# ikt-luh/Demo-Learned-Point-Cloud-Compression

Measured on AMD Instinct MI355X. Metric: point-cloud frames/sec encode+decode @1M pts, higher is better.
Workload: dtype f32

## Files before the change

demo-learned-point-cloud-compression_amd/csrc/codec.hip:

```cpp
#include "common.h"

#include <string.h>

#include <algorithm>
#include <atomic>
#include <chrono>
#include <deque>
#include <exception>
#include <new>
#include <map>
#include <memory>
#include <string>
#include <condition_variable>
#include <functional>
#include <mutex>
#include <thread>
#include <vector>

namespace {

double now_s() {
  return std::chrono::duration<double>(std::chrono::steady_clock::now().time_since_epoch()).count();
}

constexpr int64_t kHashBuildMax = 60000;
constexpr int64_t kMaxLatentRows = (int64_t)1 << 27;
constexpr int64_t kEarlyZSymbols = (int64_t)1 << 22;

int log2i(int ts) {
  int s = 0;
  while ((1 << s) < ts) ++s;
  return s;
}

struct Tensor {
  int dtype = 0;
  std::vector<int64_t> dims;
  const uint8_t* data = nullptr;
  size_t nbytes = 0;
  int64_t numel() const {
    int64_t n = 1;
    for (int64_t d : dims) n *= d;
    return n;
  }
  const float* f32() const { return reinterpret_cast<const float*>(data); }
  const int32_t* i32() const { return reinterpret_cast<const int32_t*>(data); }
};

struct DevPool {
  struct Block {
    char* p;
    size_t cap, off;
  };
  std::vector<Block> blocks;
  void reset() {
    if (blocks.size() > 32) {
      size_t total = 0;
      for (auto& b : blocks) total += b.cap;
      release();
      char* p = nullptr;
      if (hipMalloc((void**)&p, total) == hipSuccess) blocks.push_back({p, total, 0});
    }
    for (auto& b : blocks) b.off = 0;
  }
  void* alloc(size_t bytes) {
    bytes = (std::max<size_t>(bytes, 1) + 255) & ~(size_t)255;
    for (auto& b : blocks)
      if (b.cap - b.off >= bytes) {
        void* r = b.p + b.off;
        b.off += bytes;
        return r;
      }
    const size_t cap = std::max<size_t>(bytes, (size_t)64 << 20);
    char* p = nullptr;
    if (hipMalloc((void**)&p, cap) != hipSuccess) {
      pcc_set_error("codec pool: hipMalloc(%zu) failed", cap);
      return nullptr;
    }
    blocks.push_back({p, cap, bytes});
    return p;
  }
  void release() {
    for (auto& b : blocks) (void)hipFree(b.p);
// ... 41 lines not shown
  uint32_t* keep = nullptr;
  int32_t* keep_remap = nullptr;
};

struct Feat {
  CS* cs = nullptr;
  float* f = nullptr;
  int c = 0;
  const uint32_t* rows = nullptr;
};

}

struct PccWorkers {
  std::vector<std::thread> th;
  std::vector<std::function<void()>> job;
  std::vector<char> busy;
  std::mutex m;
  std::condition_variable cv_job, cv_done;
  bool stop = false;

  void ensure(int n) {
    std::unique_lock<std::mutex> lk(m);
    while ((int)th.size() < n) {
      const int i = (int)th.size();
      job.resize((size_t)i + 1);
      busy.resize((size_t)i + 1, 0);
      th.emplace_back([this, i]() {
        std::unique_lock<std::mutex> l(m);
        for (;;) {
          cv_job.wait(l, [&] { return stop || busy[i]; });
          if (stop) return;
          std::function<void()> f = std::move(job[i]);
          l.unlock();
          try {
            f();
          } catch (...) {
          }
          l.lock();
          busy[i] = 0;
          cv_done.notify_all();
        }
      });
    }
  }
  void run(int i, std::function<void()> f) {
    {
      std::lock_guard<std::mutex> lk(m);
      job[i] = std::move(f);
      busy[i] = 1;
    }
    cv_job.notify_all();
  }
  void wait_range(int lo, int hi) {
    std::unique_lock<std::mutex> lk(m);
    cv_done.wait(lk, [&] {
      for (int i = lo; i < hi && i < (int)busy.size(); ++i)
        if (busy[i]) return false;
      return true;
    });
  }
  void wait_all() {
    std::unique_lock<std::mutex> lk(m);
    cv_done.wait(lk, [&] {
      for (char b : busy)
        if (b) return false;
      return true;
    });
  }
  ~PccWorkers() {
    {
      std::lock_guard<std::mutex> lk(m);
      stop = true;
    }
    cv_job.notify_all();
    for (auto& t : th)
      if (t.joinable()) t.join();
  }
};

struct WorkersGuard {
  PccWorkers* w;
  ~WorkersGuard() { if (w) w->wait_all(); }
};

struct pcc_codec {
  pcc_ctx* ctx = nullptr;
  int device = 0;
  std::vector<uint8_t> blob;
  std::map<std::string, Tensor> t;
  std::map<std::string, float*> dev;
  int c_y = 32, c_z = 32;
  PccRansTables* gc_tables = nullptr;
  PccRansTables* eb_tables = nullptr;
  int container_version = 0;
  int seek_points = 0;
  struct ScaleSlot {
    std::vector<double> key;
    float* dev = nullptr;
    size_t cap = 0;
  } scale_slot[2];
  pcc_rans_dev *gc_dev = nullptr, *eb_dev = nullptr;
  PccWorkers workers;
  DevPool pool;
  Pinned pin_keys, pin_occ, pin_zsym, pin_ysym, pin_yidx, pin_flag, pin_dec, pin_up;
  hipStream_t up_stream = nullptr;
  hipStream_t side_stream = nullptr;
  pcc_ctx* side_ctx = nullptr;
  hipEvent_t up_done = nullptr;
  std::vector<hipEvent_t> events;
  size_t events_used = 0;
  std::deque<CS> sets;
  std::vector<std::vector<uint8_t>> out;
  int32_t* rec_coords = nullptr;
  float* rec_colors = nullptr;
  int64_t rec_n = 0;
  std::vector<int64_t> rec_offsets;
  bool rec_i16 = false;
  int16_t* rec_xyz16 = nullptr;
  float* rec_rgbp = nullptr;
  Pinned pin_out;
  hipEvent_t out_pts = nullptr;
  std::atomic<int> widen_status{0};
};

void octree_root(uint64_t first, uint64_t last, int key_shift, int* depth, int32_t origin[3]) {
  const uint64_t mask48 = ((uint64_t)1 << 48) - 1;
  const uint64_t a = (first & mask48) >> key_shift, b = (last & mask48) >> key_shift;
  const uint64_t diff = a ^ b;
  int d = 1;
  if (diff) d = (63 - __builtin_clzll(diff)) / 3 + 1;
  const uint64_t corner = (a >> (3 * d)) << (3 * d);
  const int bias = 32768 >> (key_shift / 3);
  auto compact = [](uint64_t v) {
    int r = 0;
    for (int i = 0; i < 16; ++i) r |= (int)((v >> (3 * i)) & 1) << i;
    return r;
  };
  *depth = d;
  origin[0] = compact(corner >> 2) - bias;
  origin[1] = compact(corner >> 1) - bias;
  origin[2] = compact(corner) - bias;
}


namespace {

#define CODEC_ALLOC(var, type, count)                                        \
  type* var = (type*)cd->pool.alloc(sizeof(type) * (size_t)(count));         \
  if (!var) return PCC_E_NOMEM

const Tensor* find(pcc_codec* cd, const std::string& name) {
  auto it = cd->t.find(name);
  if (it == cd->t.end()) {
    pcc_set_error("codec: checkpoint has no tensor '%s'", name.c_str());
    return nullptr;
  }
  return &it->second;
}

CS* new_set(pcc_codec* cd, uint64_t* keys, int64_t n, int stride, int n_batch) {
  cd->sets.emplace_back();
  CS* s = &cd->sets.back();
  s->keys = keys;
  s->n = n;
  s->stride = stride;
  s->n_batch = n_batch;
  return s;
}

int keys_of(pcc_codec* cd, CS* s, uint64_t** out);

int offsets_of(pcc_codec* cd, CS* s, const std::vector<int64_t>** out) {
  if (s->offsets.empty()) {
    if (s->n_batch == 1) {
      s->offsets = {0, s->n};
    } else if (s->gen_parent) {
      const std::vector<int64_t>* po;
      PCC_TRY(offsets_of(cd, s->gen_parent, &po));
      s->offsets.resize(po->size());
      for (size_t i = 0; i < po->size(); ++i) s->offsets[i] = 8 * (*po)[i];
    } else {
      s->offsets.assign((size_t)s->n_batch + 1, 0);
      PCC_TRY(pcc_batch_offsets(cd->ctx, s->keys, s->n, s->n_batch, s->offsets.data()));
    }
  }
  *out = &s->offsets;
  return PCC_OK;
}

int down_of(pcc_codec* cd, CS* s) {
  if (s->down) return PCC_OK;
// ... 333 lines not shown
}

struct Reader {
  const uint8_t* p;
  int64_t len, pos = 0;
  bool bad = false;
  int32_t be32() {
    if (pos + 4 > len) { bad = true; return 0; }
    const uint32_t u = ((uint32_t)p[pos] << 24) | ((uint32_t)p[pos + 1] << 16) | ((uint32_t)p[pos + 2] << 8) | p[pos + 3];
    pos += 4;
    return (int32_t)u;
  }
  double be_f64() {
    if (pos + 8 > len) { bad = true; return 0; }
    uint64_t u = 0;
    for (int i = 0; i < 8; ++i) u = (u << 8) | p[pos + i];
    pos += 8;
    double d;
    memcpy(&d, &u, 8);
    return d;
  }
  const uint8_t* bytes(int64_t n) {
    if (n < 0 || pos + n > len) { bad = true; return nullptr; }
    const uint8_t* r = p + pos;
    pos += n;
    return r;
  }
};

int rans_encode_grow(const int32_t* sym, const int32_t* idx, int64_t n, const Tensor* cdf, const Tensor* len,
                     const Tensor* off, std::vector<uint8_t>* out) {
  int64_t cap = 2 * n + 4096, got = 0;
  int rc = PCC_OK;
  for (int attempt = 0; attempt < 2; ++attempt) {
    out->resize((size_t)cap);
    rc = pcc_rans_encode(sym, idx, n, cdf->i32(), (int)cdf->dims[1], len->i32(), off->i32(), (int)cdf->dims[0],
                         out->data(), cap, &got);
    if (rc != PCC_E_NOMEM) break;
    cap = 48 * n + 4096;
  }
  if (rc == PCC_OK) out->resize((size_t)got);
  return rc;
}

}


static void warm_copy_paths(pcc_codec* cd) {
  hipStream_t st = cd->ctx->stream;
  const size_t big = (size_t)1 << 20;
  uint8_t *d = nullptr, *h = nullptr;
  if (hipMalloc((void**)&d, 2 * big) != hipSuccess) return;
  if (hipHostMalloc((void**)&h, 2 * big, hipHostMallocDefault) == hipSuccess) {
    for (int rep = 0; rep < 2; ++rep) {
      for (size_t bytes : {(size_t)64, (size_t)4096, (size_t)65536, big}) {
        for (int k = 0; k < 4; ++k) {
          (void)hipMemcpyAsync(h + (size_t)k * (big / 4), d + (size_t)k * (big / 4), std::min(bytes, big / 4), hipMemcpyDeviceToHost, st);
          (void)hipMemcpyAsync(d + big + (size_t)k * (big / 4), h + big + (size_t)k * (big / 4), std::min(bytes, big / 4),
                               hipMemcpyHostToDevice, st);
        }
        (void)hipMemcpy2DAsync(h, big / 4, d, big / 4, std::min(bytes, big / 4), 3, hipMemcpyDeviceToHost, st);
        (void)hipMemcpy2DAsync(h + big, big / 4, d + big, big / 4, std::min(bytes, big / 4) / 2 + 1, 3, hipMemcpyDeviceToHost, st);
      }
      (void)hipMemsetAsync(d, 0, 4096, st);
      (void)hipMemcpyAsync(d + big, d, 65536, hipMemcpyDeviceToDevice, st);
    }
    (void)hipStreamSynchronize(st);
    (void)hipHostFree(h);
  }
  (void)hipFree(d);
  (void)hipGetLastError();
}

extern "C" pcc_codec* pcc_codec_create(const void* h_ckpt, size_t n, int device, void* stream) {
  if (!h_ckpt || n < 8 || memcmp(h_ckpt, "PCCW", 4) != 0) {
    pcc_set_error("pcc_codec_create: not a PCCW checkpoint blob");
    return nullptr;
  }
  pcc_ctx* ctx = pcc_create(device, stream);
  if (!ctx) return nullptr;
  pcc_codec* cd = new pcc_codec();
  cd->ctx = ctx;
  cd->device = device;
  cd->blob.assign((const uint8_t*)h_ckpt, (const uint8_t*)h_ckpt + n);
  const uint8_t* p = cd->blob.data();
  size_t pos = 4;
  auto fail = [&](const char* why) -> pcc_codec* {
    pcc_set_error("pcc_codec_create: malformed checkpoint (%s)", why);
    pcc_destroy(cd->ctx);
    delete cd;
    return nullptr;
  };
  uint32_t count;
  memcpy(&count, p + pos, 4);
  pos += 4;
  for (uint32_t i = 0; i < count; ++i) {
    if (pos + 2 > n) return fail("truncated");
    uint16_t nl;
    memcpy(&nl, p + pos, 2);
    pos += 2;
    if (pos + nl + 2 > n) return fail("truncated name");
    std::string name((const char*)p + pos, nl);
    pos += nl;
    Tensor t;
    t.dtype = p[pos];
    const int nd = p[pos + 1];
    pos += 2;
    if (pos + 4 * (size_t)nd + 8 > n) return fail("truncated dims");
    for (int d = 0; d < nd; ++d) {
      uint32_t v;
      memcpy(&v, p + pos, 4);
      pos += 4;
      t.dims.push_back(v);
    }
    uint64_t nb;
    memcpy(&nb, p + pos, 8);
    pos += 8;
    pos = (pos + 7) & ~(size_t)7;
    if (pos + nb > n || nb != (uint64_t)t.numel() * 4) return fail("bad tensor size");
    t.data = p + pos;
    t.nbytes = nb;
    pos = (pos + nb + 7) & ~(size_t)7;
    cd->t[name] = t;
  }
  for (auto& kv : cd->t) {
    const std::string& k = kv.first;
    const bool is_wb = (k.size() > 7 && k.compare(k.size() - 7, 7, ".weight") == 0) ||
                       (k.size() > 5 && k.compare(k.size() - 5, 5, ".bias") == 0);
    const bool is_tab = k == "entropy_bottleneck.medians" || k == "gaussian_conditional.scale_table";
    if ((!is_wb && !is_tab) || k.compare(0, 8, "scale_nn") == 0 || kv.second.dtype != 0) continue;
    float* d = nullptr;
    if (hipMalloc((void**)&d, std::max<size_t>(kv.second.nbytes, 4)) != hipSuccess ||
        hipMemcpy(d, kv.second.data, kv.second.nbytes, hipMemcpyHostToDevice) != hipSuccess) {
      pcc_set_error("pcc_codec_create: upload of '%s' failed", k.c_str());
      pcc_destroy(cd->ctx);
      delete cd;
      return nullptr;
    }
    cd->dev[k] = d;
  }
  for (auto& kv : cd->t) {
    const std::string& k = kv.first;
    const Tensor& t = kv.second;
    if (k.size() <= 7 || k.compare(k.size() - 7, 7, ".weight") != 0 || t.dtype != 0 || t.dims.size() != 3) continue;
    const std::string layer = k.substr(0, k.size() - 7);
    const bool is_up = layer.find(".up") != std::string::npos;
    if (is_up && t.dims[0] == 8 && t.dims[1] == 32 && t.dims[2] == 32 && cd->dev.count(k))
      (void)pcc_conv_prepare(ctx, cd->dev[k], 8, 32, 32);
    if (!is_up && (t.dims[0] == 27 || t.dims[0] == 8) && t.dims[1] % 16 == 0 && t.dims[2] % 16 == 0 && t.dims[1] <= 128 &&
        t.dims[2] <= 256 && cd->dev.count(k)) {
      if (pcc_conv_prepare(ctx, cd->dev[k], (int)t.dims[0], (int)t.dims[1], (int)t.dims[2]) != PCC_OK) {
        for (auto& d : cd->dev) (void)hipFree(d.second);
        pcc_destroy(cd->ctx);
        delete cd;
        return nullptr;
      }
    }
    if (is_up && layer.compare(0, 4, "g_s.") == 0 && t.dims[0] == 8 && t.dims[1] == 32 && t.dims[2] == 32 &&
        cd->t.count(layer + ".bias")) {
      std::vector<float> wp((size_t)t.numel()), bp(32);
      const float* bsrc = cd->t[layer + ".bias"].f32();
      for (int64_t r = 0; r < 8 * 32; ++r)
        for (int j = 0; j < 32; ++j) wp[(size_t)r * 32 + j] = t.f32()[r * 32 + pcc_conv16_perm(j)];
      for (int j = 0; j < 32; ++j) bp[j] = bsrc[pcc_conv16_perm(j)];
      float *dw = nullptr, *db = nullptr;
      if (hipMalloc((void**)&dw, wp.size() * 4) != hipSuccess || hipMalloc((void**)&db, 128) != hipSuccess ||
// ... 14 lines not shown
  }
  static const char* need[] = {"g_a.conv0.weight", "g_a.conv3.weight", "h_a.conv0.weight", "h_s.conv0.weight",
                               "g_s.color.weight", "entropy_bottleneck.quantized_cdf",
                               "gaussian_conditional.quantized_cdf", "gaussian_conditional.scale_table",
                               "entropy_bottleneck.medians", "entropy_model.offsets_ab", "entropy_model.eps"};
  for (const char* k : need)
    if (!cd->t.count(k)) {
      pcc_set_error("pcc_codec_create: checkpoint has no tensor '%s'", k);
      for (auto& kv : cd->dev) (void)hipFree(kv.second);
      pcc_destroy(cd->ctx);
      delete cd;
      return nullptr;
    }
  cd->c_y = (int)cd->t["g_a.conv3.weight"].dims[2];
  cd->c_z = (int)cd->t["entropy_bottleneck.medians"].dims[0];
  {
    const Tensor *gc_cdf = find(cd, "gaussian_conditional.quantized_cdf"), *gc_len = find(cd, "gaussian_conditional.cdf_length"),
                 *gc_off = find(cd, "gaussian_conditional.offset");
    if (gc_cdf && gc_len && gc_off)
      cd->gc_tables = pcc_rans_tables_build(gc_cdf->i32(), (int)gc_cdf->dims[1], gc_len->i32(), gc_off->i32(),
                                            (int)gc_cdf->dims[0]);
    if (!cd->gc_tables) {
      for (auto& kv : cd->dev) (void)hipFree(kv.second);
      pcc_destroy(cd->ctx);
      delete cd;
      return nullptr;
    }
    const Tensor *eb_cdf = find(cd, "entropy_bottleneck.quantized_cdf"), *eb_len = find(cd, "entropy_bottleneck.cdf_length"),
                 *eb_off = find(cd, "entropy_bottleneck.offset");
    cd->gc_dev = pcc_rans_dev_create(gc_cdf->i32(), (int)gc_cdf->dims[1], gc_len->i32(), gc_off->i32(), (int)gc_cdf->dims[0]);
    if (eb_cdf && eb_len && eb_off)
      cd->eb_tables = pcc_rans_tables_build(eb_cdf->i32(), (int)eb_cdf->dims[1], eb_len->i32(), eb_off->i32(),
                                            (int)eb_cdf->dims[0]);
    if (eb_cdf && eb_len && eb_off)
      cd->eb_dev = pcc_rans_dev_create(eb_cdf->i32(), (int)eb_cdf->dims[1], eb_len->i32(), eb_off->i32(), (int)eb_cdf->dims[0]);
  }
  warm_copy_paths(cd);
  return cd;
}

extern "C" int pcc_codec_set_seek_points(pcc_codec* cd, int pieces) {
  PCC_REQUIRE(cd, PCC_E_ARG, "pcc_codec_set_seek_points: null codec");
  PCC_REQUIRE(pieces == 0 || (pieces >= 2 && pieces <= 64), PCC_E_ARG, "pcc_codec_set_seek_points: %d pieces (0, or 2 .. 64)", pieces);
  cd->seek_points = pieces;
  return PCC_OK;
}

static void seek_indexes(int64_t n, int pieces, std::vector<int64_t>* out) {
  out->clear();
  if (pieces < 2 || n < 65536) return;
  for (int k = 1; k < pieces; ++k) {
    const int64_t i = (n * k / pieces) & ~(int64_t)63;
    if (i > 0 && i < n && (out->empty() || i > out->back())) out->push_back(i);
  }
}

extern "C" int pcc_codec_set_container_version(pcc_codec* cd, int version) {
  PCC_REQUIRE(cd, PCC_E_ARG, "pcc_codec_set_container_version: null codec");
  PCC_REQUIRE(version == 0 || version == 1, PCC_E_ARG, "pcc_codec_set_container_version: version %d (0 or 1)", version);
  PCC_REQUIRE(version == 0 || (cd->gc_dev && cd->eb_dev), PCC_E_ARG,
              "pcc_codec_set_container_version: the checkpoint's CDF tables have no device form");
  cd->container_version = version;
  return PCC_OK;
}

extern "C" void pcc_codec_destroy(pcc_codec* cd) {
  if (!cd) return;
  if (cd->ctx) (void)pcc_sync(cd->ctx);
  for (auto& kv : cd->dev) (void)hipFree(kv.second);
  for (auto& sl : cd->scale_slot)
    if (sl.dev) (void)hipFree(sl.dev);
  pcc_rans_tables_free(cd->gc_tables);
  pcc_rans_tables_free(cd->eb_tables);
  pcc_rans_dev_destroy(cd->gc_dev);
  pcc_rans_dev_destroy(cd->eb_dev);
  cd->pool.release();
  if (cd->up_stream) {
    (void)hipStreamSynchronize(cd->up_stream);
    (void)hipStreamDestroy(cd->up_stream);
  }
  if (cd->side_ctx) pcc_destroy(cd->side_ctx);
  if (cd->side_stream) (void)hipStreamDestroy(cd->side_stream);
  if (cd->up_done) (void)hipEventDestroy(cd->up_done);
  if (cd->out_pts) (void)hipEventDestroy(cd->out_pts);
  for (hipEvent_t e : cd->events) (void)hipEventDestroy(e);
  for (Pinned* p : {&cd->pin_keys, &cd->pin_occ, &cd->pin_zsym, &cd->pin_ysym, &cd->pin_yidx, &cd->pin_flag, &cd->pin_dec,
                    &cd->pin_up, &cd->pin_out})
    p->release();
  pcc_destroy(cd->ctx);
  delete cd;
}

extern "C" pcc_ctx* pcc_codec_ctx(pcc_codec* cd) { return cd ? cd->ctx : nullptr; }

#define PCC_MAX_FRAMES_ARG 32
struct FrameTab {
  const void* pts[PCC_MAX_FRAMES_ARG];
  const void* cols[PCC_MAX_FRAMES_ARG];
  long long off[PCC_MAX_FRAMES_ARG + 1];
  int nf, pts_i16, cols_f64;
};
struct HostFrames {
  const void* const* pts;
  const void* const* cols;
};

__device__ __forceinline__ int frame_of(const FrameTab& t, long long i) {
  int f = 0;
  while (f + 1 < t.nf && i >= t.off[f + 1]) ++f;
  return f;
}

__global__ __launch_bounds__(256) void k_frames_keys(FrameTab t, int64_t n, uint64_t* __restrict__ keys,
                                                     int32_t* __restrict__ flag) {
  const int64_t i = (int64_t)blockIdx.x * blockDim.x + threadIdx.x;
  if (i >= n) return;
  const int f = frame_of(t, i);
  const int64_t j = i - t.off[f];
  int x, y, z;
  if (t.pts_i16) {
    const int16_t* p = (const int16_t*)t.pts[f] + 3 * j;
    x = p[0]; y = p[1]; z = p[2];
  } else {
    const int32_t* p = (const int32_t*)t.pts[f] + 3 * j;
    x = p[0]; y = p[1]; z = p[2];
    const bool bad = (x < -32768) | (x > 32767) | (y < -32768) | (y > 32767) | (z < -32768) | (z > 32767);
    if (bad) atomicOr(flag, 1);
  }
  keys[i] = pcc_morton(f, x, y, z);
}

__global__ void k_frame_end_keys(FrameTab t, const uint64_t* __restrict__ keys, uint64_t* __restrict__ out) {
  const int f = threadIdx.x;
  if (f >= t.nf) return;
  const bool any = t.off[f + 1] > t.off[f];
  out[2 * f] = any ? keys[t.off[f]] : 0ull;
  out[2 * f + 1] = any ? keys[t.off[f + 1] - 1] : 0ull;
}

__global__ __launch_bounds__(256) void k_frames_feats(FrameTab t, const uint32_t* __restrict__ perm, int64_t n,
                                                      float4* __restrict__ feats) {
  const int64_t i = (int64_t)blockIdx.x * blockDim.x + threadIdx.x;
  if (i >= n) return;
  const long long src = perm[i];
  const int f = frame_of(t, src);
  const int64_t j = src - t.off[f];
  float r, g, b;
  if (t.cols_f64) {
    const double* c = (const double*)t.cols[f] + 3 * j;
    r = (float)c[0]; g = (float)c[1]; b = (float)c[2];
  } else {
    const float* c = (const float*)t.cols[f] + 3 * j;
    r = c[0]; g = c[1]; b = c[2];
  }
  feats[i] = make_float4(1.0f, r, g, b);
}

struct UploadPiece {
  size_t off;
  const void* src;
  size_t count;
  int f64;
};
constexpr int kUploadThreads = 4;
constexpr size_t kUploadPieceBytes = (size_t)1 << 20;

static void upload_pieces(std::vector<UploadPiece>* out, size_t base, const void* src, size_t n_bytes_out, int f64) {
  for (size_t o = 0; o < n_bytes_out; o += kUploadPieceBytes) {
    const size_t len = std::min(kUploadPieceBytes, n_bytes_out - o);
    if (f64)
      out->push_back({base + o, (const double*)src + o / 4, len / 4, 1});
    else
      out->push_back({base + o, (const char*)src + o, len, 0});
  }
}

static void upload_run(pcc_codec* cd, const std::vector<UploadPiece>& pieces, char* stage, char* dev, hipStream_t stream,
                       std::atomic<int>* status) {
  cd->workers.ensure(kUploadThreads);
  const int device = cd->device;
  for (int w = 0; w < kUploadThreads; ++w)
    cd->workers.run(w, [&pieces, stage, dev, stream, status, device, w]() {
      if (stream && hipSetDevice(device) != hipSuccess) status->store(1);
      for (size_t i = (size_t)w; i < pieces.size(); i += kUploadThreads) {
        const UploadPiece& p = pieces[i];
        size_t bytes = p.count;
        if (p.f64) {
          float* d = (float*)(stage + p.off);
          const double* sp = (const double*)p.src;
          for (size_t j = 0; j < p.count; ++j) d[j] = (float)sp[j];
          bytes = p.count * 4;
        } else {
          memcpy(stage + p.off, p.src, p.count);
        }
        if (stream && hipMemcpyAsync(dev + p.off, stage + p.off, bytes, hipMemcpyHostToDevice, stream) != hipSuccess)
          status->store(1);
      }
    });
}

static int begin_call(pcc_codec* cd) {
  PCC_HIP(hipSetDevice(cd->device));
  PCC_TRY(pcc_sync(cd->ctx));
  if (cd->up_stream) PCC_HIP(hipStreamSynchronize(cd->up_stream));
  if (cd->side_stream) PCC_HIP(hipStreamSynchronize(cd->side_stream));
  cd->pool.reset();
  cd->events_used = 0;
  cd->sets.clear();
  return PCC_OK;
}

template <class F>
static int timed(double* clock, F&& stage) {
  const double t0 = now_s();
  const int rc = stage();
  *clock += now_s() - t0;
  return rc;
}

namespace {

int pack_octree(const uint8_t* occ, const std::vector<int64_t>& level_n, int depth, int64_t n, const int32_t origin[3],
                int64_t nodes, std::vector<uint8_t>* out) {
  const int64_t zero = 0;
  const int32_t org0[3] = {0, 0, 0};
  out->resize((size_t)(64 + 2 * nodes + 16));
  int64_t len = 0;
  const int rc = pcc_octree_pack(n ? occ : nullptr, n ? level_n.data() : &zero, n ? depth : 0, n, n ? origin : org0,
                                 out->data(), (int64_t)out->size(), &len);
  out->resize((size_t)(rc == PCC_OK ? len : 0));
  return rc;
}

struct GeoSlotEncoder {
  struct Frame {
    int64_t n = 0, occ_off = 0, occ_len = 0, cap = 0;
    int depth = 0;
    int32_t origin[3] = {0, 0, 0};
    std::vector<int64_t> level_n;
    std::vector<uint8_t> v2;
    struct Part {
      int64_t n = 0, occ_off = 0, nodes = 0;
      std::vector<int64_t> level_n;
    };
    int K = 1;
    int counts_at = 0;
    std::vector<Part> parts;
  };
  static constexpr int kCounts = 20;
  pcc_codec* cd = nullptr;
  const CS* ycs = nullptr;
  const std::vector<int64_t>* yoffs = nullptr;
  const uint64_t* ends = nullptr;
  std::vector<Frame> fr;
  int n_blocks = 0;
  bool small = false, queued = false, async = false;
  hipEvent_t ev = nullptr;
  double dev_s = 0, host_s = 0;
  void init(pcc_codec* c, int nf, const CS* y, const std::vector<int64_t>* offs, const std::vector<uint64_t>& root_keys) {
    cd = c;
    ycs = y;
    yoffs = offs;
    ends = root_keys.data();
    fr.resize((size_t)nf);
    small = (int)root_keys.size() == 2 * nf;
    for (int f = 0; f < nf; ++f) small &= (*offs)[f + 1] - (*offs)[f] <= pcc_octree_small_max();
  }
  int64_t layout(const uint64_t* keys_h) {
    int64_t total = 0;
    for (int f = 0; f < (int)fr.size(); ++f) {
      Frame& g = fr[f];
      g.n = (*yoffs)[f + 1] - (*yoffs)[f];
      g.occ_off = total;
      if (small) {
        g.K = g.n >= PCC_OCTREE_V3_MIN_LEAVES ? pcc_octree_parts_for(g.n) : 1;
        g.counts_at = n_blocks;
        n_blocks += g.K;
      }
      if (g.n == 0) continue;
      octree_root(small ? ends[2 * f] : keys_h[(*yoffs)[f]], small ? ends[2 * f + 1] : keys_h[(*yoffs)[f + 1] - 1], 9,
                  &g.depth, g.origin);
// ... 109 lines not shown
      if (g.K == 1 || g.parts.empty()) {
        PCC_TRY(pack_octree(cd->pin_occ.p + g.occ_off, g.level_n, g.depth, g.n, g.origin, g.occ_len, &blobs[f]));
        continue;
      }
      std::vector<std::vector<uint8_t>> pb((size_t)g.K);
      std::vector<int> prc((size_t)g.K, PCC_OK);
      std::vector<std::string> perr((size_t)g.K);
      auto pack_part = [&](int k) {
        const Frame::Part& pt = g.parts[(size_t)k];
        prc[(size_t)k] = pack_octree(cd->pin_occ.p + pt.occ_off, pt.level_n, g.depth, pt.n, g.origin, pt.nodes,
                                     &pb[(size_t)k]);
        if (prc[(size_t)k] != PCC_OK) perr[(size_t)k] = pcc_last_error();
      };
      if (threads) {
        cd->workers.ensure(g.K - 1);
        for (int k = 1; k < g.K; ++k) cd->workers.run(k - 1, [&pack_part, k]() { pack_part(k); });
        pack_part(0);
        cd->workers.wait_all();
      } else {
        for (int k = 0; k < g.K; ++k) pack_part(k);
      }
      for (int k = 0; k < g.K; ++k)
        if (prc[(size_t)k] != PCC_OK) {
          pcc_set_error("pcc_encode_gop (geometry, frame %d part %d): %s", f, k, perr[(size_t)k].c_str());
          return prc[(size_t)k];
        }
      int64_t tot = 64 + 4 * g.K;
      for (const auto& b : pb) tot += (int64_t)b.size();
      blobs[f].resize((size_t)tot);
      int64_t len = 0;
      PCC_TRY(pcc_octree_join_parts(g.depth, g.origin, g.n, pb.data(), g.K, blobs[f].data(), tot, &len));
      blobs[f].resize((size_t)len);
    }
    host_s = now_s() - t;
    return PCC_OK;
  }
};

struct EncodeCall {
  pcc_codec* cd;
  pcc_ctx* ctx;
  hipStream_t st;
  const double* h_q;
  int n_frames, n_q, cy, cz;
  bool v1 = false;
  pcc_ctx* side = nullptr;
  double ts[8] = {0, 0, 0, 0, 0, 0, 0, 0};
  Feat x, y, z, z_hat, gp;
  View yv, zv;
  int64_t ny = 0, nz = 0;
  float* ys_f = nullptr;
  int32_t* zsym_dev = nullptr;
  const std::vector<int64_t>* yoffs = nullptr;
  std::vector<uint64_t> root_keys;
  std::vector<int64_t> counts[3];
  GeoSlotEncoder geo;
  int64_t cap_y = 0, cap_z = 0;
  long long* d_lens = nullptr;
  hipEvent_t z_done = nullptr;
  const Tensor *eb_cdf = nullptr, *eb_len = nullptr, *eb_off = nullptr;
  const Tensor *gc_cdf = nullptr, *gc_len = nullptr, *gc_off = nullptr;
  std::vector<std::vector<uint8_t>> blobs, y_strings;
  std::vector<uint8_t> z_string, head_done;
  std::vector<int64_t> seek_idx;
  std::vector<std::vector<uint64_t>> seek_state;
  std::vector<std::vector<int64_t>> seek_word;
  int n_chunks = 1;
  std::vector<int64_t> bound;
  std::vector<hipEvent_t> evc;
  std::vector<int> rcq;
  std::vector<std::string> errq;
  double helper_z_s = 0;
  EncodeCall(pcc_codec* c, int nf, const double* q, int nq)
      : cd(c), ctx(c->ctx), st(c->ctx->stream), h_q(q), n_frames(nf), n_q(nq), cy(c->c_y), cz(c->c_z),
        blobs((size_t)nf), y_strings((size_t)nq), head_done((size_t)nq, 0) {}
  int unpack(int64_t n, const int32_t* d_coords, const float* d_feats, const FrameTab* frames_in, const HostFrames* host) {
    CODEC_ALLOC(keys, uint64_t, n);
    CODEC_ALLOC(flag, int32_t, 1);
    CODEC_ALLOC(perm, uint32_t, n);
    CODEC_ALLOC(f, float, 4 * n);
    PCC_HIP(hipMemsetAsync(flag, 0, 4, st));
    FrameTab ftab;
    const FrameTab* frames = frames_in;
    std::vector<UploadPiece> col_pieces;
    std::atomic<int> up_status{0};
    WorkersGuard up_guard{nullptr};
    if (host) {
      if (!cd->up_stream) {
        PCC_HIP(hipStreamCreateWithFlags(&cd->up_stream, hipStreamNonBlocking));
        PCC_HIP(hipEventCreateWithFlags(&cd->up_done, hipEventDisableTiming));
      }
      PCC_HIP(hipStreamSynchronize(cd->up_stream));
      ftab = *frames_in;
      const size_t pb = ftab.pts_i16 ? 6 : 12, cb = 12;
      char* dp = (char*)cd->pool.alloc((size_t)n * pb + 256 * (size_t)ftab.nf);
      char* dc = (char*)cd->pool.alloc((size_t)n * cb + 256 * (size_t)ftab.nf);
      if (!dp || !dc) return PCC_E_NOMEM;
      std::vector<UploadPiece> pt_pieces;
      size_t po = 0, co = 0;
      for (int f = 0; f < ftab.nf; ++f) {
        const size_t nf = (size_t)(ftab.off[f + 1] - ftab.off[f]);
        ftab.pts[f] = dp + po;
        upload_pieces(&pt_pieces, po, host->pts[f], nf * pb, 0);
        po += (nf * pb + 255) & ~(size_t)255;
      }
      const size_t pts_bytes = po;
      for (int f = 0; f < ftab.nf; ++f) {
        const size_t nf = (size_t)(ftab.off[f + 1] - ftab.off[f]);
        ftab.cols[f] = dc + co;
        upload_pieces(&col_pieces, co, host->cols[f], nf * cb, ftab.cols_f64);
        co += (nf * cb + 255) & ~(size_t)255;
      }
      ftab.cols_f64 = 0;
      PCC_TRY(cd->pin_up.ensure(pts_bytes + co));
      up_guard.w = &cd->workers;
      upload_run(cd, pt_pieces, (char*)cd->pin_up.p, dp, cd->up_stream, &up_status);
      cd->workers.wait_all();
      PCC_REQUIRE(up_status.load() == 0, PCC_E_HIP, "pcc_encode_gop_host_frames: upload of the frame arrays failed");
      hipEvent_t pts_up;
      PCC_TRY(call_event(cd, &pts_up));
      PCC_HIP(hipEventRecord(pts_up, cd->up_stream));
      PCC_HIP(hipStreamWaitEvent(st, pts_up, 0));
      upload_run(cd, col_pieces, (char*)cd->pin_up.p + pts_bytes, dc, cd->up_stream, &up_status);
      frames = &ftab;
    }
    if (frames) {
      hipLaunchKernelGGL(k_frames_keys, dim3((unsigned)((n + 255) / 256)), dim3(256), 0, st, *frames, n, keys, flag);
      PCC_CHECK_LAUNCH();
    } else {
      PCC_TRY(pcc_morton_keys_batch(ctx, d_coords, n, n_frames, keys, flag));
    }
    PCC_TRY(pcc_sort_pairs_bytes(ctx, keys, perm, n, 0x3Fu | (n_frames > 1 ? 0x40u : 0u) | (n_frames > 256 ? 0x80u : 0u)));
    PCC_TRY(cd->pin_flag.ensure(64 + 16 * PCC_MAX_FRAMES_ARG));
    PCC_HIP(hipMemcpyAsync(cd->pin_flag.p, flag, 4, hipMemcpyDeviceToHost, st));
    if (frames) {
      CODEC_ALLOC(ends, uint64_t, 2 * PCC_MAX_FRAMES_ARG);
      hipLaunchKernelGGL(k_frame_end_keys, dim3(1), dim3(PCC_MAX_FRAMES_ARG), 0, st, *frames, (const uint64_t*)keys, ends);
      PCC_CHECK_LAUNCH();
      PCC_HIP(hipMemcpyAsync(cd->pin_flag.p + 64, ends, (size_t)16 * frames->nf, hipMemcpyDeviceToHost, st));
    }
    int dup = 0;
    std::vector<int64_t> level_n(5, 0);
    PCC_TRY(pcc_level_counts(ctx, keys, n, 0, 5, level_n.data(), &dup));
    PCC_HIP(hipStreamSynchronize(st));
    PCC_REQUIRE(*(int32_t*)cd->pin_flag.p == 0, PCC_E_RANGE,
                "pcc_encode_gop: coordinate outside [-32768,32767] or batch index outside [0, n_frames)");
    PCC_REQUIRE(!dup, PCC_E_DUP, "pcc_encode_gop: duplicate coordinates");
    if (frames) root_keys.assign((const uint64_t*)(cd->pin_flag.p + 64), (const uint64_t*)(cd->pin_flag.p + 64) + 2 * frames->nf);
    x = {new_set(cd, keys, n, 1, n_frames), f, 4};
    x.cs->down_counts = level_n;
    if (host) {
      int32_t* nbr0;
      PCC_TRY(nbr27_of(cd, x.cs, &nbr0));
      cd->workers.wait_all();
      up_guard.w = nullptr;
      PCC_REQUIRE(up_status.load() == 0, PCC_E_HIP, "pcc_encode_gop_host_frames: upload of the frame arrays failed");
      PCC_HIP(hipEventRecord(cd->up_done, cd->up_stream));
      PCC_HIP(hipStreamWaitEvent(st, cd->up_done, 0));
    }
    if (frames) {
      hipLaunchKernelGGL(k_frames_feats, dim3((unsigned)((n + 255) / 256)), dim3(256), 0, st, *frames,
                         (const uint32_t*)perm, n, (float4*)f);
      PCC_CHECK_LAUNCH();
      return PCC_OK;
    }
    return pcc_gather_rows(ctx, d_feats, perm, n, 16, f);
  }
  int analysis(int64_t* h_k) {
    Feat h = x;
    for (int j = 0; j < 3; ++j) {
      const std::vector<int64_t>* offs;
      PCC_TRY(offsets_of(cd, h.cs, &offs));
      for (int f = 0; f < n_frames; ++f) counts[j].push_back((*offs)[f + 1] - (*offs)[f]);
      Feat a, b;
      PCC_TRY(conv3(cd, "g_a.conv" + std::to_string(j), h, 1, &a));
      PCC_TRY(down2(cd, "g_a.down" + std::to_string(j), a, 1, &b));
      h = b;
    }
    PCC_TRY(conv3(cd, "g_a.conv3", h, 0, &y));
    if (h_k)
      for (int s = 0; s < 3; ++s)
        for (int f = 0; f < n_frames; ++f) h_k[s * n_frames + f] = counts[2 - s][f];
    ny = y.cs->n;
    PCC_TRY(view_of(cd, y.cs, &yv));
    CODEC_ALLOC(ys, float, std::max<int64_t>(ny, 1) * cy);
    ys_f = ys;
    if (ny > 0) PCC_TRY(pcc_gather_rows(ctx, y.f, yv.perm, ny, 4 * cy, ys_f));
    return offsets_of(cd, y.cs, &yoffs);
  }
  int start_side() {
    geo.init(cd, n_frames, y.cs, yoffs, root_keys);
    v1 = cd->container_version == 1;
    if (v1) PCC_TRY(side_of(cd, &side));
    if (side && geo.small) {
      hipEvent_t ev_y;
      PCC_TRY(call_event(cd, &ev_y));
      PCC_HIP(hipEventRecord(ev_y, st));
      PCC_HIP(hipStreamWaitEvent(side->stream, ev_y, 0));
      PCC_TRY(geo.device_half(side));
    }
    return PCC_OK;
  }
  int hyper_analysis() {
    Feat a, b;
    PCC_TRY(conv3(cd, "h_a.conv0", y, 1, &a));
    PCC_TRY(down2(cd, "h_a.down0", a, 1, &b));
    return down2(cd, "h_a.down1", b, 0, &z);
  }
  int factorized() {
    nz = z.cs->n;
    PCC_TRY(view_of(cd, z.cs, &zv));
    CODEC_ALLOC(zs_f, float, std::max<int64_t>(nz, 1) * cz);
    CODEC_ALLOC(zsym, int32_t, std::max<int64_t>(nz, 1) * cz);
    CODEC_ALLOC(zhat_rows, float, std::max<int64_t>(nz, 1) * cz);
    zsym_dev = zsym;
    PCC_TRY(cd->pin_zsym.ensure((size_t)std::max<int64_t>(nz, 1) * cz * 4));
    if (nz > 0) {
      PCC_TRY(pcc_gather_rows(ctx, z.f, zv.perm, nz, 4 * cz, zs_f));
      PCC_TRY(pcc_factorized_quant(ctx, zs_f, nz, cz, cd->dev["entropy_bottleneck.medians"], zsym, zhat_rows));
      if (!v1) PCC_HIP(hipMemcpyAsync(cd->pin_zsym.p, zsym, (size_t)nz * cz * 4, hipMemcpyDeviceToHost, st));
    }
    float* zf;
    PCC_TRY(rows_to_tensor(cd, zv, zhat_rows, cz, &zf));
    z_hat = {z.cs, zf, cz};
    const int64_t per_y = (int64_t)cy * ny, nzs = (int64_t)cz * nz;
    if (v1) {
      PCC_REQUIRE(cd->gc_dev && cd->eb_dev, PCC_E_ARG, "pcc_encode_gop: container version 1 without device CDF tables");
      cap_y = std::min<int64_t>(pcc_rans_dev_bound(per_y), (6 * per_y + 65536) / 4 * 4);
      cap_z = std::min<int64_t>(pcc_rans_dev_bound(nzs), (6 * nzs + 65536) / 4 * 4);
      PCC_TRY(cd->pin_ysym.ensure((size_t)cap_y * n_q + (size_t)cap_z + 256));
      d_lens = (long long*)cd->pool.alloc(sizeof(long long) * (size_t)(n_q + 1));
      if (!d_lens) return PCC_E_NOMEM;
      if (side) {
        hipEvent_t ev_z;
        PCC_TRY(call_event(cd, &ev_z));
        PCC_TRY(call_event(cd, &z_done));
        PCC_HIP(hipEventRecord(ev_z, st));
        PCC_HIP(hipStreamWaitEvent(side->stream, ev_z, 0));
        PCC_TRY(pcc_rans_encode_dev_async(side, cd->eb_dev, zsym_dev, nullptr, std::max<int64_t>(nz, 1), nzs, 1,
                                          cd->pin_ysym.p + (size_t)cap_y * n_q, cap_z, d_lens + n_q, 0));
        PCC_HIP(hipEventRecord(z_done, side->stream));
// ... 1160 lines not shown
```

Before: 118.9.

## Pipeline host staging and H2D copies per block across upload workers

Replaces the per-piece upload with a block plan: each 4 MiB block is split into slices staged by all worker threads, and a block's H2D copy is issued, in order, as soon as all its slices are staged. The compute stream is released after the last points block rather than after a full wait_all barrier, and colour staging continues without a second dispatch. The f64-to-f32 colour conversion now uses AVX/SSE2 intrinsics. An optional env-gated trace records timings. The cost is added mutex and atomic coordination and larger copy granularity.

Result: no change. 118.2 (-0.6%).

```diff
diff --git a/demo-learned-point-cloud-compression_amd/csrc/codec.hip b/demo-learned-point-cloud-compression_amd/csrc/codec.hip
--- a/demo-learned-point-cloud-compression_amd/csrc/codec.hip
+++ b/demo-learned-point-cloud-compression_amd/csrc/codec.hip
@@ -1,4 +1,5 @@
 #include "common.h"
+#include "upload_stage.h"
 
 #include <string.h>
 
@@ -206,6 +207,16 @@
 struct WorkersGuard {
   PccWorkers* w;
   ~WorkersGuard() { if (w) w->wait_all(); }
+};
+
+struct UploadTrace {
+  struct Slice { int thread; double begin, end; };
+  struct Block { int thread; double call, ret; };
+  double t0 = 0;
+  std::vector<Slice> slices;
+  std::vector<Block> blocks;
+  std::vector<double> run_at, woke_at;
+  std::vector<hipEvent_t> ev;
 };
 
 struct pcc_codec {
@@ -232,6 +243,7 @@
   hipStream_t side_stream = nullptr;
   pcc_ctx* side_ctx = nullptr;
   hipEvent_t up_done = nullptr;
+  std::unique_ptr<UploadTrace> up_trace;
   std::vector<hipEvent_t> events;
   size_t events_used = 0;
   std::deque<CS> sets;
@@ -731,6 +743,8 @@
   pcc_codec* cd = new pcc_codec();
   cd->ctx = ctx;
   cd->device = device;
+  if (const char* e = getenv("PCC_UPLOAD_TRACE"))
+    if (e[0] && e[0] != '0') cd->up_trace.reset(new UploadTrace());
   cd->blob.assign((const uint8_t*)h_ckpt, (const uint8_t*)h_ckpt + n);
   const uint8_t* p = cd->blob.data();
   size_t pos = 4;
@@ -911,6 +925,8 @@
   if (cd->side_ctx) pcc_destroy(cd->side_ctx);
   if (cd->side_stream) (void)hipStreamDestroy(cd->side_stream);
   if (cd->up_done) (void)hipEventDestroy(cd->up_done);
+  if (cd->up_trace)
+    for (hipEvent_t e : cd->up_trace->ev) (void)hipEventDestroy(e);
   if (cd->out_pts) (void)hipEventDestroy(cd->out_pts);
   for (hipEvent_t e : cd->events) (void)hipEventDestroy(e);
   for (Pinned* p : {&cd->pin_keys, &cd->pin_occ, &cd->pin_zsym, &cd->pin_ysym, &cd->pin_yidx, &cd->pin_flag, &cd->pin_dec,
@@ -985,47 +1001,133 @@
   feats[i] = make_float4(1.0f, r, g, b);
 }
 
-struct UploadPiece {
-  size_t off;
-  const void* src;
-  size_t count;
-  int f64;
+constexpr int kUploadThreads = kPccUploadThreads;
+constexpr size_t kUploadBlockBytes = kPccUploadBlockBytes;
+static_assert(kUploadThreads >= 1 && kUploadThreads <= 8, "a GPU host grants a caller few CPUs");
+static_assert(kUploadBlockBytes % 256 == 0, "blocks begin where frames may: at multiples of 256");
+
+struct UploadRun {
+  PccUpPlan plan;
+  char* stage = nullptr;
+  char* dev[2] = {nullptr, nullptr};
+  hipStream_t stream = nullptr;
+  hipStream_t compute = nullptr;
+  hipEvent_t pts_up = nullptr;
+  int n_pts_blocks = 0;
+  int device = 0;
+  std::unique_ptr<std::atomic<int>[]> left;
+  std::mutex m;
+  std::condition_variable cv;
+  std::vector<char> staged;
+  size_t next_block = 0;
+  bool pts_sent = false;
+  std::atomic<int>* status = nullptr;
+  UploadTrace* trace = nullptr;
+
+  void send_staged() {
+    while (next_block < plan.blocks.size() && staged[next_block]) {
+      const size_t b = next_block++;
+      const PccUpBlock& bl = plan.blocks[b];
+      if (trace) {
+        if (b == 0 && hipEventRecord(trace->ev[0], stream) != hipSuccess) status->store(1);
+        trace->blocks[b].call = now_s() - trace->t0;
+      }
+      if (hipMemcpyAsync(dev[bl.group] + bl.rel, stage + bl.off, bl.bytes, hipMemcpyHostToDevice, stream) != hipSuccess)
+        status->store(1);
+      if (trace) {
+        trace->blocks[b].ret = now_s() - trace->t0;
+        if (hipEventRecord(trace->ev[1 + b], stream) != hipSuccess) status->store(1);
+      }
+      if ((int)b + 1 == n_pts_blocks) {
+        if (hipEventRecord(pts_up, stream) != hipSuccess || hipStreamWaitEvent(compute, pts_up, 0) != hipSuccess) status->store(1);
+        pts_sent = true;
+        cv.notify_all();
+      }
+    }
+  }
+  void work(int w) {
+    if (trace) trace->woke_at[(size_t)w] = now_s() - trace->t0;
+    if (hipSetDevice(device) != hipSuccess) status->store(1);
+    for (size_t i = (size_t)w; i < plan.slices.size(); i += (size_t)kUploadThreads) {
+      const PccUpSlice& sl = plan.slices[i];
+      const double t_begin = trace ? now_s() : 0;
+      pcc_up_stage(stage, sl);
+      if (trace) trace->slices[i] = {w, t_begin - trace->t0, now_s() - trace->t0};
+      if (left[(size_t)sl.block].fetch_sub(1, std::memory_order_acq_rel) == 1) {
+        std::lock_guard<std::mutex> lk(m);
+        staged[(size_t)sl.block] = 1;
+        if (trace) trace->blocks[(size_t)sl.block].thread = w;
+        send_staged();
+      }
+    }
+  }
+  int start(pcc_codec* cd) {
+    const size_t nb = plan.blocks.size();
+    left.reset(new std::atomic<int>[nb]);
+    for (size_t b = 0; b < nb; ++b) left[b].store(plan.blocks[b].n_slices);
+    staged.assign(nb, 0);
+    device = cd->device;
+    trace = cd->up_trace.get();
+    if (trace) {
+      while (trace->ev.size() < nb + 1) {
+        hipEvent_t e;
+        PCC_HIP(hipEventCreate(&e));
+        trace->ev.push_back(e);
+      }
+      trace->slices.assign(plan.slices.size(), {0, 0, 0});
+      trace->blocks.assign(nb, {0, 0, 0});
+      trace->run_at.assign((size_t)kUploadThreads, 0);
+      trace->woke_at.assign((size_t)kUploadThreads, 0);
+      trace->t0 = now_s();
+    }
+    cd->workers.ensure(kUploadThreads);
+    for (int w = 0; w < kUploadThreads; ++w) {
+      if (trace) trace->run_at[(size_t)w] = now_s() - trace->t0;
+      cd->workers.run(w, [this, w]() { work(w); });
+    }
+    return PCC_OK;
+  }
+  void wait_points() {
+    std::unique_lock<std::mutex> lk(m);
+    cv.wait(lk, [&] { return pts_sent; });
+  }
 };
-constexpr int kUploadThreads = 4;
-constexpr size_t kUploadPieceBytes = (size_t)1 << 20;
-
-static void upload_pieces(std::vector<UploadPiece>* out, size_t base, const void* src, size_t n_bytes_out, int f64) {
-  for (size_t o = 0; o < n_bytes_out; o += kUploadPieceBytes) {
-    const size_t len = std::min(kUploadPieceBytes, n_bytes_out - o);
-    if (f64)
-      out->push_back({base + o, (const double*)src + o / 4, len / 4, 1});
-    else
-      out->push_back({base + o, (const char*)src + o, len, 0});
-  }
-}
-
-static void upload_run(pcc_codec* cd, const std::vector<UploadPiece>& pieces, char* stage, char* dev, hipStream_t stream,
-                       std::atomic<int>* status) {
-  cd->workers.ensure(kUploadThreads);
-  const int device = cd->device;
-  for (int w = 0; w < kUploadThreads; ++w)
-    cd->workers.run(w, [&pieces, stage, dev, stream, status, device, w]() {
-      if (stream && hipSetDevice(device) != hipSuccess) status->store(1);
-      for (size_t i = (size_t)w; i < pieces.size(); i += kUploadThreads) {
-        const UploadPiece& p = pieces[i];
-        size_t bytes = p.count;
-        if (p.f64) {
-          float* d = (float*)(stage + p.off);
-          const double* sp = (const double*)p.src;
-          for (size_t j = 0; j < p.count; ++j) d[j] = (float)sp[j];
-          bytes = p.count * 4;
-        } else {
-          memcpy(stage + p.off, p.src, p.count);
-        }
-        if (stream && hipMemcpyAsync(dev + p.off, stage + p.off, bytes, hipMemcpyHostToDevice, stream) != hipSuccess)
-          status->store(1);
-      }
-    });
+
+static void upload_trace_print(const UploadRun& u) {
+  const UploadTrace& t = *u.trace;
+  const PccUpPlan& p = u.plan;
+  fprintf(stderr, "# upload trace: %zu blocks of up to %zu bytes, %zu slices, %zu threads; host times in us since the first run()\n",
+          p.blocks.size(), (size_t)kUploadBlockBytes, p.slices.size(), t.woke_at.size());
+  for (size_t w = 0; w < t.woke_at.size(); ++w) {
+    double busy[2] = {0, 0}, moved[2] = {0, 0}, last = 0;
+    int cnt[2] = {0, 0};
+    for (size_t i = 0; i < p.slices.size(); ++i)
+      if (t.slices[i].thread == (int)w) {
+        const int g = p.blocks[(size_t)p.slices[i].block].group;
+        busy[g] += t.slices[i].end - t.slices[i].begin;
+        moved[g] += (double)p.slices[i].bytes * (p.slices[i].f64 ? 3 : 2);
+        ++cnt[g];
+        last = std::max(last, t.slices[i].end);
+      }
+    fprintf(stderr, "worker %zu  run() %6.1f  woke %6.1f (wake-up %5.1f)  points %3d slices %7.1f us %6.1f GB/s   colours %3d slices %7.1f us %6.1f GB/s   last slice ends %7.1f\n",
+            w, t.run_at[w] * 1e6, t.woke_at[w] * 1e6, (t.woke_at[w] - t.run_at[w]) * 1e6, cnt[0], busy[0] * 1e6,
+            busy[0] > 0 ? moved[0] / busy[0] * 1e-9 : 0.0, cnt[1], busy[1] * 1e6, busy[1] > 0 ? moved[1] / busy[1] * 1e-9 : 0.0, last * 1e6);
+  }
+  std::vector<double> first(p.blocks.size(), 1e30), lastv(p.blocks.size(), 0);
+  for (size_t i = 0; i < p.slices.size(); ++i) {
+    first[(size_t)p.slices[i].block] = std::min(first[(size_t)p.slices[i].block], t.slices[i].begin);
+    lastv[(size_t)p.slices[i].block] = std::max(lastv[(size_t)p.slices[i].block], t.slices[i].end);
+  }
+  fprintf(stderr, "block group    bytes slices  staging begin      end   copy call   return (host cost)  by   engine done  since previous  (engine times: us after the first copy command reached it)\n");
+  float prev = 0;
+  for (size_t b = 0; b < p.blocks.size(); ++b) {
+    float ms = 0;
+    (void)hipEventElapsedTime(&ms, t.ev[0], t.ev[1 + b]);
+    fprintf(stderr, "%5zu %-7s %8zu %4d  %13.1f %8.1f  %10.1f %8.1f (%6.1f)  w%d  %11.1f %11.1f\n", b, p.blocks[b].group ? "colours" : "points",
+            p.blocks[b].bytes, p.blocks[b].n_slices, first[b] * 1e6, lastv[b] * 1e6, t.blocks[b].call * 1e6, t.blocks[b].ret * 1e6,
+            (t.blocks[b].ret - t.blocks[b].call) * 1e6, t.blocks[b].thread, ms * 1e3, (ms - prev) * 1e3);
+    prev = ms;
+  }
 }
 
 static int begin_call(pcc_codec* cd) {
@@ -1301,8 +1403,8 @@
     PCC_HIP(hipMemsetAsync(flag, 0, 4, st));
     FrameTab ftab;
     const FrameTab* frames = frames_in;
-    std::vector<UploadPiece> col_pieces;
     std::atomic<int> up_status{0};
+    UploadRun up;
     WorkersGuard up_guard{nullptr};
     if (host) {
       if (!cd->up_stream) {
@@ -1315,32 +1417,39 @@
       char* dp = (char*)cd->pool.alloc((size_t)n * pb + 256 * (size_t)ftab.nf);
       char* dc = (char*)cd->pool.alloc((size_t)n * cb + 256 * (size_t)ftab.nf);
       if (!dp || !dc) return PCC_E_NOMEM;
-      std::vector<UploadPiece> pt_pieces;
+      std::vector<PccUpArray> pt_arrays, col_arrays;
       size_t po = 0, co = 0;
       for (int f = 0; f < ftab.nf; ++f) {
         const size_t nf = (size_t)(ftab.off[f + 1] - ftab.off[f]);
         ftab.pts[f] = dp + po;
-        upload_pieces(&pt_pieces, po, host->pts[f], nf * pb, 0);
+        pt_arrays.push_back({host->pts[f], po, nf * pb, 0});
         po += (nf * pb + 255) & ~(size_t)255;
       }
       const size_t pts_bytes = po;
       for (int f = 0; f < ftab.nf; ++f) {
         const size_t nf = (size_t)(ftab.off[f + 1] - ftab.off[f]);
         ftab.cols[f] = dc + co;
-        upload_pieces(&col_pieces, co, host->cols[f], nf * cb, ftab.cols_f64);
+        col_arrays.push_back({host->cols[f], co, nf * cb, ftab.cols_f64});
         co += (nf * cb + 255) & ~(size_t)255;
       }
       ftab.cols_f64 = 0;
       PCC_TRY(cd->pin_up.ensure(pts_bytes + co));
+      pcc_up_plan_add(&up.plan, pt_arrays.data(), ftab.nf, 0, 0, kUploadBlockBytes, kUploadThreads);
+      up.n_pts_blocks = (int)up.plan.blocks.size();
+      pcc_up_plan_add(&up.plan, col_arrays.data(), ftab.nf, 1, pts_bytes, kUploadBlockBytes, kUploadThreads);
+      up.stage = (char*)cd->pin_up.p;
+      up.dev[0] = dp;
+      up.dev[1] = dc;
+      up.stream = cd->up_stream;
+      up.compute = st;
+      up.status = &up_status;
+      PCC_TRY(call_event(cd, &up.pts_up));
       up_guard.w = &cd->workers;
-      upload_run(cd, pt_pieces, (char*)cd->pin_up.p, dp, cd->up_stream, &up_status);
-      cd->workers.wait_all();
-      PCC_REQUIRE(up_status.load() == 0, PCC_E_HIP, "pcc_encode_gop_host_frames: upload of the frame arrays failed");
-      hipEvent_t pts_up;
-      PCC_TRY(call_event(cd, &pts_up));
-      PCC_HIP(hipEventRecord(pts_up, cd->up_stream));
-      PCC_HIP(hipStreamWaitEvent(st, pts_up, 0));
-      upload_run(cd, col_pieces, (char*)cd->pin_up.p + pts_bytes, dc, cd->up_stream, &up_status);
+      PCC_TRY(up.start(cd));
+      if (up.n_pts_blocks > 0) {
+        up.wait_points();
+        PCC_REQUIRE(up_status.load() == 0, PCC_E_HIP, "pcc_encode_gop_host_frames: upload of the frame arrays failed");
+      }
       frames = &ftab;
     }
     if (frames) {
@@ -1376,6 +1485,10 @@
       PCC_REQUIRE(up_status.load() == 0, PCC_E_HIP, "pcc_encode_gop_host_frames: upload of the frame arrays failed");
       PCC_HIP(hipEventRecord(cd->up_done, cd->up_stream));
       PCC_HIP(hipStreamWaitEvent(st, cd->up_done, 0));
+      if (up.trace) {
+        PCC_HIP(hipEventSynchronize(cd->up_done));
+        upload_trace_print(up);
+      }
     }
     if (frames) {
       hipLaunchKernelGGL(k_frames_feats, dim3((unsigned)((n + 255) / 256)), dim3(256), 0, st, *frames,
diff --git a/demo-learned-point-cloud-compression_amd/csrc/upload_stage.h b/demo-learned-point-cloud-compression_amd/csrc/upload_stage.h
--- /dev/null
+++ b/demo-learned-point-cloud-compression_amd/csrc/upload_stage.h
@@ -0,0 +1,107 @@
+#pragma once
+
+#include <stddef.h>
+#include <stdint.h>
+#include <string.h>
+
+#include <algorithm>
+#include <vector>
+
+#if defined(__x86_64__) || defined(__i386__)
+#include <immintrin.h>
+#endif
+
+constexpr size_t kPccUploadBlockBytes = (size_t)4 << 20;
+constexpr int kPccUploadThreads = 4;
+
+struct PccUpArray {
+  const void* src;
+  size_t off;
+  size_t bytes;
+  int f64;
+};
+struct PccUpSlice {
+  size_t off;
+  const void* src;
+  size_t bytes;
+  int f64;
+  int block;
+};
+struct PccUpBlock {
+  size_t off;
+  size_t rel;
+  size_t bytes;
+  int group;
+  int n_slices;
+};
+struct PccUpPlan {
+  std::vector<PccUpSlice> slices;
+  std::vector<PccUpBlock> blocks;
+};
+
+static inline size_t pcc_up_slice_bytes(size_t block_bytes, int n_threads) {
+  const size_t t = (size_t)std::max(n_threads, 1);
+  return ((block_bytes + t - 1) / t + 63) & ~(size_t)63;
+}
+
+static inline void pcc_up_plan_add(PccUpPlan* plan, const PccUpArray* arrays, int n_arrays, int group, size_t stage_base,
+                                   size_t block_bytes, int n_threads) {
+  size_t end = 0;
+  for (int a = 0; a < n_arrays; ++a)
+    if (arrays[a].bytes) end = arrays[a].off + arrays[a].bytes;
+  const size_t first_block = plan->blocks.size();
+  size_t k_next = 0;
+  for (int a = 0; a < n_arrays; ++a) {
+    const PccUpArray& ar = arrays[a];
+    for (size_t s = ar.off; s < ar.off + ar.bytes;) {
+      const size_t k = s / block_bytes;
+      for (; k_next <= k; ++k_next) {
+        const size_t lo = k_next * block_bytes;
+        plan->blocks.push_back({stage_base + lo, lo, std::min(block_bytes, end - lo), group, 0});
+      }
+      const size_t step = pcc_up_slice_bytes(plan->blocks[first_block + k].bytes, n_threads);
+      const size_t e = std::min({ar.off + ar.bytes, (k + 1) * block_bytes, s + step});
+      const size_t in_array = s - ar.off;
+      const void* src = ar.f64 ? (const void*)((const double*)ar.src + in_array / 4) : (const void*)((const char*)ar.src + in_array);
+      plan->slices.push_back({stage_base + s, src, e - s, ar.f64, (int)(first_block + k)});
+      ++plan->blocks[first_block + k].n_slices;
+      s = e;
+    }
+  }
+}
+
+#if defined(__x86_64__)
+__attribute__((target("avx"))) static inline void pcc_up_convert_avx(float* __restrict d, const double* __restrict s, size_t n) {
+  size_t i = 0;
+  for (; i + 8 <= n; i += 8) {
+    _mm_storeu_ps(d + i, _mm256_cvtpd_ps(_mm256_loadu_pd(s + i)));
+    _mm_storeu_ps(d + i + 4, _mm256_cvtpd_ps(_mm256_loadu_pd(s + i + 4)));
+  }
+  for (; i < n; ++i) d[i] = (float)s[i];
+}
+static inline void pcc_up_convert_sse2(float* __restrict d, const double* __restrict s, size_t n) {
+  size_t i = 0;
+  for (; i + 4 <= n; i += 4)
+    _mm_storeu_ps(d + i, _mm_movelh_ps(_mm_cvtpd_ps(_mm_loadu_pd(s + i)), _mm_cvtpd_ps(_mm_loadu_pd(s + i + 2))));
+  for (; i < n; ++i) d[i] = (float)s[i];
+}
+#endif
+
+static inline void pcc_up_convert(float* __restrict d, const double* __restrict s, size_t n) {
+#if defined(__x86_64__)
+  static const bool avx = __builtin_cpu_supports("avx");
+  if (avx)
+    pcc_up_convert_avx(d, s, n);
+  else
+    pcc_up_convert_sse2(d, s, n);
+#else
+  for (size_t i = 0; i < n; ++i) d[i] = (float)s[i];
+#endif
+}
+
+static inline void pcc_up_stage(char* stage, const PccUpSlice& sl) {
+  if (sl.f64)
+    pcc_up_convert((float*)(stage + sl.off), (const double*)sl.src, sl.bytes / 4);
+  else
+    memcpy(stage + sl.off, sl.src, sl.bytes);
+}
```
